# TravisWheelerLab/BATH

Measured on AMD Instinct MI355X. Metric: DP Gcells/s + residues/s through bathsearch pipeline at 1/2/4/8 MI355X, higher is better.
Workload: dtype u8/i16 integer scores (SSV: exact binary16), f32 Forward

## Files before the change

bath_amd/csrc/bath_common.hpp:

```cpp
#pragma once
#include <set>
#include <atomic>
#include <hip/hip_runtime.h>

#include <cstdint>
#include <chrono>
#include <cstdio>
#include <cstdlib>
#include <cstring>
#include <condition_variable>
#include <functional>
#include <mutex>
#include <string>
#include <thread>
#include <vector>

#include "bath_hip.h"
#include "bath_tilings.hpp"
#include "bath_slots.hpp"

namespace bath {

inline hipError_t allow_max_lds(const void *fn) {
  static std::mutex mu;
  static std::set<std::pair<int, const void *>> done;
  int dev = 0;
  (void)hipGetDevice(&dev);
  std::lock_guard<std::mutex> g(mu);
  if (done.count({dev, fn})) return hipSuccess;
  hipFuncAttributes at{};
  size_t fixed = 0;
  if (hipFuncGetAttributes(&at, fn) == hipSuccess) fixed = at.sharedSizeBytes; else (void)hipGetLastError();
  const hipError_t e = hipFuncSetAttribute(fn, hipFuncAttributeMaxDynamicSharedMemorySize, (int)(160 * 1024 - (int)std::min<size_t>(fixed, 96 * 1024)));
  if (e == hipSuccess) done.insert({dev, fn});
  return e;
}

constexpr int kKp = BATH_KP_AMINO;
constexpr int kRowReset = 29;
constexpr int kSsvRows = 30;
constexpr size_t kSsvLdsMax = 160 * 1024;
constexpr int kSsvMaxNodes = 2560;
constexpr int kStop = 27;
constexpr int kXaa = 26;
constexpr int kOrfBins = 2048;
constexpr int kOrfCursorStride = 32;
constexpr int kOrfMiscInts = (1 + kOrfCursorStride) * kOrfBins + 64;
constexpr int kFsMaxNodes = 64 * BATH_TILING_MAX(BATH_FS_COLUMNS);
constexpr int kCascadeMaxNodes = 64 * BATH_TILING_MAX(BATH_WAVE_COLUMNS);

#define BATH_HIP_TRY(ctx, call)                                                            \
  do {                                                                                     \
    hipError_t e_ = (call);                                                                \
    if (e_ != hipSuccess) {                                                                \
      (ctx)->set_error(std::string(#call) + ": " + hipGetErrorString(e_));                 \
      return BATH_EFAIL;                                                                   \
    }                                                                                      \
  } while (0)

struct DevBuf {
  void *p = nullptr;
  size_t cap = 0;
  hipError_t reserve(size_t bytes) {
    if (bytes <= cap) return hipSuccess;
    if (p) (void)hipFree(p);
    p = nullptr; cap = 0;
    size_t want = bytes + bytes / 4 + 256;
    hipError_t e = hipMalloc(&p, want);
    if (e == hipSuccess) cap = want;
    return e;
  }
  void release() { if (p) (void)hipFree(p); p = nullptr; cap = 0; }
  template <class T> T *as() const { return reinterpret_cast<T *>(p); }
};

struct HostBuf {
  void *p = nullptr;
  size_t cap = 0;
  bool coherent = false;
  hipError_t reserve(size_t bytes, bool want_coherent = false) {
    if (bytes <= cap && (coherent || !want_coherent)) return hipSuccess;
    if (p) (void)hipHostFree(p);
    p = nullptr; cap = 0;
    coherent = coherent || want_coherent;
    size_t want = bytes + bytes / 4 + 256;
    hipError_t e = hipHostMalloc(&p, want, coherent ? (hipHostMallocCoherent | hipHostMallocMapped | hipHostMallocPortable) : hipHostMallocDefault);
    if (e == hipSuccess) cap = want;
    return e;
  }
  void release() { if (p) (void)hipHostFree(p); p = nullptr; cap = 0; }
  template <class T> T *as() const { return reinterpret_cast<T *>(p); }
};

struct LanePool {
  std::mutex m;
  std::condition_variable cv_work, cv_done;
  std::vector<std::thread> th;
  std::function<void(int)> fn;
  int gen = 0, pending = 0, K = 0;
  bool stop = false;
  void loop(int id) {
    int seen = 0;
    for (;;) {
      std::function<void(int)> f;
      {
        std::unique_lock<std::mutex> l(m);
        cv_work.wait(l, [&] { return stop || (gen != seen && id < K); });
        if (stop) return;
        seen = gen; f = fn;
      }
      f(id);
      { std::lock_guard<std::mutex> l(m); if (--pending == 0) cv_done.notify_all(); }
    }
  }
  void run(int k, std::function<void(int)> f) {
    while ((int)th.size() < k) { const int id = (int)th.size(); th.emplace_back([this, id] { loop(id); }); }
    { std::lock_guard<std::mutex> l(m); fn = std::move(f); K = k; pending = k; gen++; }
    cv_work.notify_all();
    std::unique_lock<std::mutex> l(m);
    cv_done.wait(l, [&] { return pending == 0; });
  }
  ~LanePool() {
    { std::lock_guard<std::mutex> l(m); stop = true; }
    cv_work.notify_all();
    for (std::thread &t : th) t.join();
  }
};

struct StageTiming { const char *name; float ms; int64_t launches; };
struct KernelSpan { const char *name; hipEvent_t a, b; double cells, bytes; };

struct PipelineSurvivor {
  int64_t window;
  int64_t aa_off;
  int32_t strand, start;
  int32_t n;
  int32_t win_start = 0;
  int32_t fs_window = -1;
  int64_t fx_off = -1;
};

}

struct bath_hip_ctx;
namespace bath {
extern std::atomic<int> g_ctx_total, g_ctx_internal;
inline int host_contexts() { return g_ctx_total.load() - g_ctx_internal.load(); }
inline void mark_internal(bath_hip_ctx *c);
}
struct bath_hip_ctx {
  int device = 0;
  hipStream_t stream = nullptr;
  hipStream_t side_stream = nullptr;
  hipEvent_t ev_fork = nullptr, ev_join = nullptr;
  hipStream_t copy_stream = nullptr;
  hipDeviceProp_t prop{};
  int fs_strict = 1;
  int fs_odds = 0;
  int fs5_odds = 0;
  int fwd_group = 0;
  int fs_ensemble = 0;
  std::atomic<int64_t> fs_ens_bound_fallbacks{0}, fs_ens_overflow_fallbacks{0}, fs_ens_bytes_kept{0};
  int std_ensemble = 0;
  std::atomic<int64_t> std_ens_serial_fallbacks{0}, std_ens_twin_fallbacks{0}, std_ens_kernel_regions{0};
  int fs_serial = -1;
  uint64_t tabs_uid = 0;
  const void *tabs_ptr = nullptr;
  uint64_t fsw_pad_uid = 0;
  int orf_tables_id = -1;
  std::string err;
  void set_error(const std::string &m) { err = m; }
  std::vector<float> fsw_len_terms;
  bath::SlotArray<bath::Scratch, bath::DevBuf> scratch;
  bath::SlotArray<bath::Pinned, bath::HostBuf> stage;
  template <class T> int stage_upload(bath::Pinned slot, void *dst, const T *src, size_t n, hipStream_t s) {
    if (stage[slot].reserve(n * sizeof(T) + 64) != hipSuccess) { set_error("cannot allocate page-locked staging memory"); return BATH_EFAIL; }
    std::memcpy(stage[slot].p, src, n * sizeof(T));
    if (hipMemcpyAsync(dst, stage[slot].p, n * sizeof(T), hipMemcpyHostToDevice, s) != hipSuccess) { set_error("staging upload failed"); return BATH_EFAIL; }
    return BATH_OK;
  }
  bath::HostBuf results_pinned;
  bath_orf_result *d_records = nullptr;
  int64_t n_records = 0;
  std::vector<bath_orf> orfs;
  std::vector<bath_fs_window> fs_windows;
  bool keep_fwd_rows = false;
  const float *fwd_rows_kept = nullptr;
  const int64_t *fwd_rows_off = nullptr;
  bool fs_want_regions = false;
  std::vector<int64_t> fs_keep_xoff;
  std::vector<int32_t> fs_regions_all;
  std::vector<bath_fs_domain> fs_domains;
  std::string cigars;
  struct TraceRec { int64_t col_off; int32_t ncol, k1, i_first, win_start, orf_start, frameshift, d_i; };
  std::vector<TraceRec> tr_recs;
  std::vector<uint16_t> tr_codes;
  std::vector<float> tr_pp;
  void traces_clear() { tr_recs.clear(); tr_codes.clear(); tr_pp.clear(); tr_valid = false; }
  void trace_push(const uint16_t *codes, const float *pp, int ncol, int k1, int i_first, int win_start, int orf_start, int frameshift, int d_i) {
    tr_recs.push_back(TraceRec{(int64_t)tr_codes.size(), ncol, k1, i_first, win_start, orf_start, frameshift, d_i});
    tr_codes.insert(tr_codes.end(), codes, codes + ncol);
    if (pp) tr_pp.insert(tr_pp.end(), pp, pp + ncol); else tr_pp.insert(tr_pp.end(), (size_t)ncol, 0.0f);
    tr_valid = false;
  }
  bool tr_valid = false;
  std::vector<bath_domain_trace> tr_out;
  std::vector<int8_t> tr_st, tr_c;
  std::vector<int32_t> tr_k, tr_i;
  std::vector<bath::PipelineSurvivor> fs_std_orfs;
  const uint8_t *fs_std_pool = nullptr;
  std::vector<uint8_t> orf_aa;
  std::vector<bath_orf_work> orf_work;
  std::vector<bath_hmm_window> hmm_windows;
  std::vector<bath::StageTiming> timings;
  std::vector<hipEvent_t> ev_pool;
  std::vector<bath::KernelSpan> spans;
  std::vector<hipEvent_t> span_events;
  size_t span_events_used = 0;
  void spans_reset() { spans.clear(); span_events_used = 0; }
  int span_begin(const char *name, hipStream_t s, double cells, double bytes) {
    auto get = [&]() -> hipEvent_t {
      if (span_events_used == span_events.size()) { hipEvent_t e; if (hipEventCreate(&e) != hipSuccess) return nullptr; span_events.push_back(e); }
      return span_events[span_events_used++];
    };
    bath::KernelSpan k{name, get(), get(), cells, bytes};
    if (!k.a || !k.b) return -1;
    (void)hipEventRecord(k.a, s);
    spans.push_back(k);
    return (int)spans.size() - 1;
  }
  void span_end(int idx, hipStream_t s) { if (idx >= 0) (void)hipEventRecord(spans[(size_t)idx].b, s); }
  std::vector<bath_hip_ctx *> lanes;
  bath::LanePool *lane_pool = nullptr;
  hipEvent_t ev_lanes = nullptr;
  bath_hip_ctx *aux = nullptr;
  bath_hip_ctx *aux2 = nullptr;
  bath_hip_ctx *aux3 = nullptr;
  bool internal = false;
};

namespace bath {
inline void mark_internal(bath_hip_ctx *c) { if (c && !c->internal) { c->internal = true; g_ctx_internal.fetch_add(1); } }
}

struct SeqView {
  const uint8_t *data;
  const int64_t *off;
  const int32_t *len;
  int64_t n;
  const int32_t *context;
};

struct bath_hip_seqs {
  bath_hip_ctx *ctx = nullptr;
  int64_t n = 0;
  int64_t total = 0;
  int64_t total_aligned = 0;
  mutable int64_t cache_minlen = -1, cache_nres = 0, cache_max_orfs = 0;
  mutable int64_t ntiles = -1;
  mutable void *d_tile_desc = nullptr;
  mutable int32_t *d_tile_first = nullptr;
  bool is_part = false;
  int64_t first_window = 0;
  mutable std::vector<bath_hip_seqs *> parts;
  int32_t maxlen = 0;
  uint8_t *d_data = nullptr;
  int64_t *d_off = nullptr;
  int32_t *d_len = nullptr;
  int32_t *d_context = nullptr;
  uint8_t *d_packed = nullptr;
  int64_t *d_poff = nullptr;
  int64_t packed_bytes = 0;
  void *d_exc = nullptr;
  int64_t exc_cap = 0, n_exc = 0;
  hipEvent_t ev_upload = nullptr;
  bool upload_pending = false;
  std::vector<int64_t> h_off;
  std::vector<int32_t> h_len;
  std::vector<int32_t> h_context;
  SeqView view() const { return SeqView{d_data, d_off, d_len, n, d_context}; }
};

struct LenTables {
  int32_t maxL = -1;
  uint8_t *d_tjb = nullptr;
  int16_t *d_xwmove = nullptr;
  float   *d_pmove = nullptr;
  float   *d_nullsc = nullptr;
  float   *d_lt1 = nullptr;
  float   *d_lt2 = nullptr;
  float   *d_p1 = nullptr;
  std::vector<uint8_t> h_tjb;
  std::vector<int16_t> h_xwmove;
  std::vector<float> h_pmove, h_nullsc;
};

struct bath_hip_oprofile {
  bath_hip_ctx *ctx = nullptr;
  uint64_t uid = 0;
  int M = 0, max_length = 0, L0 = 0;
  float nj = 1.f;
  float evparam[BATH_NEVPARAM];
  float compo[BATH_K_AMINO];
  std::vector<uint8_t> rb;
  std::vector<int16_t> rw;
  std::vector<int16_t> tw;
  std::vector<float> rf, tf;
// ... 54 lines not shown
```

bath_amd/csrc/bath_profile.hip:

```cpp
#include <atomic>
#include <cctype>
#include <cmath>
#include <cstring>

#include "bath_common.hpp"
#include "host_model.hpp"

using namespace bath;

namespace bath {

static const double kLog2 = 0.69314718055994529;

double gumbel_surv(double x, double mu, double lambda) {
  double ey = -std::exp(-lambda * (x - mu));
  if (std::fabs(ey) < 5e-9) return -ey;
  return 1.0 - std::exp(ey);
}
double gumbel_invsurv(double p, double mu, double lambda) {
  double lp = (p < 5e-9) ? (std::pow(p, p) - 1) / p : std::log(-1. * std::log(1 - p));
  return mu - lp / lambda;
}
double exp_surv(double x, double mu, double lambda) { return (x < mu) ? 1.0 : std::exp(-lambda * (x - mu)); }

static inline uint8_t cost_u8(float scale, float sc) {
  float c = -1.0f * roundf(scale * sc);
  return (c > 255.) ? 255 : (uint8_t)(int)c;
}
static inline uint8_t cost_u8_biased(float scale, uint8_t bias, float sc) {
  float c = -1.0f * roundf(scale * sc);
  return (c > 255 - bias) ? 255 : (uint8_t)((int)c + bias);
}
static inline int16_t score_i16(float scale, float sc) {
  float v = roundf(scale * sc);
  if (v >= 32767.0) return 32767;
  if (v <= -32768.0) return -32768;
  return (int16_t)v;
}

void bias_filter_eo(const float *compo, float eo[kKp][2]) {
  for (int x = 0; x < 20; x++) { eo[x][0] = kAminoBg[x] / kAminoBg[x]; eo[x][1] = compo[x] / kAminoBg[x]; }
  for (int x : {20, 27, 28}) eo[x][0] = eo[x][1] = 1.0f;
  for (int x = 21; x <= 26; x++)
    for (int s = 0; s < 2; s++) {
      float num = 0.f, den = 0.f;
      for (int y = 0; y < 20; y++)
        if (amino_degen_has(x, y)) { num += (s == 0 ? kAminoBg[y] : compo[y]); den += kAminoBg[y]; }
      eo[x][s] = den > 0.f ? num / den : 0.f;
    }
}

template <class T>
static hipError_t upload(T **dst, const T *src, size_t n, hipStream_t st) {
  hipError_t e = hipMalloc((void **)dst, n * sizeof(T) + 64);
  if (e != hipSuccess) return e;
  return hipMemcpyAsync(*dst, src, n * sizeof(T), hipMemcpyHostToDevice, st);
}

int build_len_tables(const bath_hip_oprofile *om, int maxL) {
  std::lock_guard<std::mutex> lock(om->grow_mu);
  LenTables &lt = om->lt;
  if (maxL <= lt.maxL) return BATH_OK;
  bath_hip_ctx *ctx = om->ctx;
  int n = std::max(maxL, 4096) + 1;
  for (void *p : {(void *)lt.d_tjb, (void *)lt.d_xwmove, (void *)lt.d_pmove, (void *)lt.d_nullsc, (void *)lt.d_lt1, (void *)lt.d_lt2, (void *)lt.d_p1})
    if (p) om->retired.push_back(p);
  lt.d_tjb = nullptr; lt.d_xwmove = nullptr; lt.d_pmove = nullptr; lt.d_nullsc = nullptr; lt.d_lt1 = nullptr; lt.d_lt2 = nullptr; lt.d_p1 = nullptr;
  lt.h_tjb.resize(n); lt.h_xwmove.resize(n); lt.h_pmove.resize(n); lt.h_nullsc.resize(n);
  std::vector<float> lt1(n), lt2(n), p1v(n);
  for (int L = 0; L < n; L++) {
    lt.h_tjb[L] = cost_u8(om->scale_b, logf(3.0f / (float)(L + 3)));
    float pmove = (2.0f + om->nj) / ((float)L + 2.0f + om->nj);
    lt.h_pmove[L] = pmove;
    lt.h_xwmove[L] = score_i16(om->scale_w, logf(pmove));
    float p1 = (float)L / (float)(L + 1);
    p1v[L] = p1;
    lt.h_nullsc[L] = (float)((float)L * std::log((double)p1) + std::log(1. - p1));
    lt1[L] = (float)L * logf(p1);
    lt2[L] = logf((float)(1. - p1));
  }
  BATH_HIP_TRY(ctx, upload(&lt.d_tjb, lt.h_tjb.data(), n, ctx->stream));
  BATH_HIP_TRY(ctx, upload(&lt.d_xwmove, lt.h_xwmove.data(), n, ctx->stream));
  BATH_HIP_TRY(ctx, upload(&lt.d_pmove, lt.h_pmove.data(), n, ctx->stream));
  BATH_HIP_TRY(ctx, upload(&lt.d_nullsc, lt.h_nullsc.data(), n, ctx->stream));
  BATH_HIP_TRY(ctx, upload(&lt.d_lt1, lt1.data(), n, ctx->stream));
  BATH_HIP_TRY(ctx, upload(&lt.d_lt2, lt2.data(), n, ctx->stream));
  BATH_HIP_TRY(ctx, upload(&lt.d_p1, p1v.data(), n, ctx->stream));
  BATH_HIP_TRY(ctx, hipStreamSynchronize(ctx->stream));
  lt.maxL = n - 1;
  return BATH_OK;
}

}

int bath_hip_oprofile::ensure_len_tables(int maxL) const { return bath::build_len_tables(this, maxL); }


namespace bath { std::atomic<int> g_ctx_total{0}, g_ctx_internal{0}; }

extern "C" int bath_hip_init(int device, bath_hip_ctx **out) {
  *out = nullptr;
  int ndev = 0;
  if (hipGetDeviceCount(&ndev) != hipSuccess || ndev <= 0) return BATH_ENODEVICE;
  if (device < 0 || device >= ndev) return BATH_EINVAL;
  bath_hip_ctx *ctx = new bath_hip_ctx();
  ctx->device = device;
  if (const char *e = std::getenv("BATH_HIP_SYNC")) {
    static const bool once = [&] {
      (void)hipSetDevice(device);
      const unsigned fl = (e[0] == 'b') ? hipDeviceScheduleBlockingSync : (e[0] == 'y') ? hipDeviceScheduleYield : hipDeviceScheduleSpin;
      if (hipSetDeviceFlags(fl) != hipSuccess) (void)hipGetLastError();
      return true;
    }();
    (void)once;
  }
  if (hipSetDevice(device) != hipSuccess || hipGetDeviceProperties(&ctx->prop, device) != hipSuccess ||
      hipStreamCreateWithFlags(&ctx->stream, hipStreamNonBlocking) != hipSuccess) {
    delete ctx;
    return BATH_ENODEVICE;
  }
  bath::g_ctx_total.fetch_add(1);
  *out = ctx;
  return BATH_OK;
}

extern "C" void bath_hip_finalize(bath_hip_ctx *ctx) {
  if (!ctx) return;
  bath::g_ctx_total.fetch_sub(1);
  if (ctx->internal) bath::g_ctx_internal.fetch_sub(1);
  (void)hipSetDevice(ctx->device);
  (void)hipStreamSynchronize(ctx->stream);
  delete ctx->lane_pool; ctx->lane_pool = nullptr;
  for (bath_hip_ctx *lane : ctx->lanes) bath_hip_finalize(lane);
  ctx->lanes.clear();
  if (ctx->ev_lanes) (void)hipEventDestroy(ctx->ev_lanes);
  if (ctx->aux) { bath_hip_finalize(ctx->aux); ctx->aux = nullptr; }
  if (ctx->aux2) { bath_hip_finalize(ctx->aux2); ctx->aux2 = nullptr; }
  if (ctx->aux3) { bath_hip_finalize(ctx->aux3); ctx->aux3 = nullptr; }
  for (auto &b : ctx->scratch) b.release();
  for (auto &b : ctx->stage) b.release();
  ctx->results_pinned.release();
  for (auto e : ctx->ev_pool) (void)hipEventDestroy(e);
  for (auto e : ctx->span_events) (void)hipEventDestroy(e);
  if (ctx->ev_fork) (void)hipEventDestroy(ctx->ev_fork);
  if (ctx->ev_join) (void)hipEventDestroy(ctx->ev_join);
  if (ctx->copy_stream) (void)hipStreamDestroy(ctx->copy_stream);
  if (ctx->side_stream) (void)hipStreamDestroy(ctx->side_stream);
  (void)hipStreamDestroy(ctx->stream);
  delete ctx;
}

extern "C" int bath_hip_trim(bath_hip_ctx *ctx) {
  if (!ctx) return BATH_EINVAL;
  BATH_HIP_TRY(ctx, hipSetDevice(ctx->device));
  BATH_HIP_TRY(ctx, hipStreamSynchronize(ctx->stream));
  delete ctx->lane_pool; ctx->lane_pool = nullptr;
  for (bath_hip_ctx *lane : ctx->lanes) bath_hip_finalize(lane);
  ctx->lanes.clear();
  if (ctx->aux) { bath_hip_finalize(ctx->aux); ctx->aux = nullptr; }
  if (ctx->aux2) { bath_hip_finalize(ctx->aux2); ctx->aux2 = nullptr; }
  if (ctx->aux3) { bath_hip_finalize(ctx->aux3); ctx->aux3 = nullptr; }
  if (ctx->copy_stream) { (void)hipStreamSynchronize(ctx->copy_stream); (void)hipStreamDestroy(ctx->copy_stream); ctx->copy_stream = nullptr; }
  if (ctx->side_stream) {
    (void)hipStreamSynchronize(ctx->side_stream); (void)hipStreamDestroy(ctx->side_stream); ctx->side_stream = nullptr;
    if (ctx->ev_fork) { (void)hipEventDestroy(ctx->ev_fork); ctx->ev_fork = nullptr; }
    if (ctx->ev_join) { (void)hipEventDestroy(ctx->ev_join); ctx->ev_join = nullptr; }
  }
  ctx->fs_std_orfs.clear(); ctx->fs_std_pool = nullptr; ctx->fs_keep_xoff.clear(); ctx->fs_regions_all.clear();
  ctx->d_records = nullptr; ctx->n_records = 0;
  return BATH_OK;
}

extern "C" const char *bath_hip_last_error(const bath_hip_ctx *ctx) { return ctx ? ctx->err.c_str() : "no context"; }

extern "C" int bath_hip_synchronize(bath_hip_ctx *ctx) {
  BATH_HIP_TRY(ctx, hipSetDevice(ctx->device));
  BATH_HIP_TRY(ctx, hipStreamSynchronize(ctx->stream));
  return BATH_OK;
}

extern "C" void *bath_hip_stream(bath_hip_ctx *ctx) { return (void *)ctx->stream; }
extern "C" int bath_hip_kernel_times(bath_hip_ctx *ctx, int max, bath_kernel_time *out) {
  if (!ctx || !out) return 0;
  int n = 0;
  for (const bath_hip_ctx *c : {(const bath_hip_ctx *)ctx, (const bath_hip_ctx *)ctx->aux, (const bath_hip_ctx *)ctx->aux2, (const bath_hip_ctx *)ctx->aux3}) {
    if (!c) continue;
    for (const bath::KernelSpan &k : c->spans) {
      float ms = 0.f;
      if (hipEventSynchronize(k.b) != hipSuccess || hipEventElapsedTime(&ms, k.a, k.b) != hipSuccess) continue;
      int i = 0;
      while (i < n && out[i].name != k.name) i++;
      if (i == n) { if (n == max) continue; out[n++] = bath_kernel_time{k.name, 0.f, 0, 0.0, 0.0}; }
      out[i].ms += ms; out[i].launches++; out[i].cells += k.cells; out[i].bytes += k.bytes;
    }
  }
  return n;
}
extern "C" int bath_hip_set_fs_serial(bath_hip_ctx *ctx, int on) {
  if (!ctx) return BATH_EINVAL;
  ctx->fs_serial = on < 0 ? -1 : (on ? 1 : 0);
  return BATH_OK;
}

extern "C" int bath_hip_set_fs_strict(bath_hip_ctx *ctx, int on) {
  if (!ctx) return BATH_EINVAL;
  ctx->fs_strict = on ? 1 : 0;
  if (!on && ctx->aux3) { bath_hip_finalize(ctx->aux3); ctx->aux3 = nullptr; }
  for (bath_hip_ctx *l : ctx->lanes) l->fs_strict = ctx->fs_strict;
  return BATH_OK;
}

extern "C" int bath_hip_set_fwd_group(bath_hip_ctx *ctx, int mode) {
  if (!ctx) return BATH_EINVAL;
  if (mode < 0 || mode > 2) { ctx->set_error("bath_hip_set_fwd_group: mode must be 0, 1 or 2"); return BATH_EINVAL; }
  ctx->fwd_group = mode;
  for (bath_hip_ctx *l : ctx->lanes) l->fwd_group = mode;
  return BATH_OK;
}

extern "C" int bath_hip_set_fs_odds(bath_hip_ctx *ctx, int on) {
  if (!ctx) return BATH_EINVAL;
  ctx->fs_odds = on ? 1 : 0;
  for (bath_hip_ctx *l : ctx->lanes) l->fs_odds = ctx->fs_odds;
  return BATH_OK;
}

extern "C" int bath_hip_set_fs5_odds(bath_hip_ctx *ctx, int on) {
  if (!ctx) return BATH_EINVAL;
  ctx->fs5_odds = on ? 1 : 0;
  for (bath_hip_ctx *l : ctx->lanes) l->fs5_odds = ctx->fs5_odds;
  return BATH_OK;
}

extern "C" int bath_hip_set_fs_ensemble(bath_hip_ctx *ctx, int mode) {
  if (!ctx) return BATH_EINVAL;
  if (mode != BATH_ENSEMBLE_SERIAL && mode != BATH_ENSEMBLE_STREAMS_HOST && mode != BATH_ENSEMBLE_STREAMS_DEVICE) { ctx->set_error("bath_hip_set_fs_ensemble: unknown mode " + std::to_string(mode)); return BATH_EINVAL; }
  ctx->fs_ensemble = mode;
  for (bath_hip_ctx *l : ctx->lanes) l->fs_ensemble = mode;
  return BATH_OK;
}

extern "C" int bath_hip_set_std_ensemble(bath_hip_ctx *ctx, int mode) {
  if (!ctx) return BATH_EINVAL;
  if (mode != BATH_ENSEMBLE_SERIAL && mode != BATH_ENSEMBLE_STREAMS_HOST && mode != BATH_ENSEMBLE_STREAMS_DEVICE) { ctx->set_error("bath_hip_set_std_ensemble: unknown mode " + std::to_string(mode)); return BATH_EINVAL; }
  ctx->std_ensemble = mode;
  for (bath_hip_ctx *l : ctx->lanes) l->std_ensemble = mode;
  if (ctx->aux) ctx->aux->std_ensemble = mode;
  return BATH_OK;
}

extern "C" int bath_hip_std_ensemble_counters(bath_hip_ctx *ctx, int64_t *serial_fallbacks, int64_t *twin_fallbacks, int64_t *kernel_regions) {
  if (!ctx) return BATH_EINVAL;
  int64_t s = 0, t = 0, k = 0;
  for (const bath_hip_ctx *c : {(const bath_hip_ctx *)ctx, (const bath_hip_ctx *)ctx->aux}) {
    if (!c) continue;
    s += c->std_ens_serial_fallbacks.load(); t += c->std_ens_twin_fallbacks.load(); k += c->std_ens_kernel_regions.load();
  }
  if (serial_fallbacks) *serial_fallbacks = s;
  if (twin_fallbacks) *twin_fallbacks = t;
  if (kernel_regions) *kernel_regions = k;
  return BATH_OK;
}

extern "C" int bath_hip_fs_ensemble_counters(bath_hip_ctx *ctx, int64_t *bound_fallbacks, int64_t *overflow_fallbacks, int64_t *matrix_bytes_kept) {
  if (!ctx) return BATH_EINVAL;
  int64_t b = 0, o = 0, k = 0;
  for (const bath_hip_ctx *c : {(const bath_hip_ctx *)ctx, (const bath_hip_ctx *)ctx->aux2}) {
    if (!c) continue;
    b += c->fs_ens_bound_fallbacks.load(); o += c->fs_ens_overflow_fallbacks.load(); k += c->fs_ens_bytes_kept.load();
  }
  if (bound_fallbacks) *bound_fallbacks = b;
  if (overflow_fallbacks) *overflow_fallbacks = o;
  if (matrix_bytes_kept) *matrix_bytes_kept = k;
  return BATH_OK;
}

extern "C" int bath_selftest_compute_units(const bath_hip_ctx *ctx) { return ctx ? ctx->prop.multiProcessorCount : 0; }


extern "C" void bath_hip_oprofile_destroy(bath_hip_oprofile *om) {
  if (!om) return;
  for (void *p : {(void *)om->d_emit, (void *)om->d_ssv, (void *)om->d_msv, (void *)om->d_rb, (void *)om->d_rw, (void *)om->d_tw, (void *)om->d_rf, (void *)om->d_tf,
                  (void *)om->d_bias_eo, (void *)om->d_compo_terms, (void *)om->d_vit_rw, (void *)om->d_vit_tw2, (void *)om->d_vit_rank, (void *)om->lt.d_tjb, (void *)om->lt.d_xwmove, (void *)om->lt.d_pmove,
                  (void *)om->lt.d_nullsc, (void *)om->lt.d_lt1, (void *)om->lt.d_lt2, (void *)om->lt.d_p1, (void *)om->d_cons, (void *)om->d_msc, (void *)om->d_tsc, (void *)om->d_rfb, (void *)om->d_tfb})
    if (p) (void)hipFree(p);
  for (void *p : om->retired) (void)hipFree(p);
  delete om;
}

extern "C" int bath_hip_oprofile_set_consensus(bath_hip_oprofile *om, const char *consensus) {
  if (!om || !consensus) return BATH_EINVAL;
  bath_hip_ctx *ctx = om->ctx;
  static const char syms[] = "ACDEFGHIKLMNPQRSTVWY-BJZOUX*~";
  om->consensus.assign((size_t)om->M + 2, ' ');
  om->cons_digital.assign((size_t)om->M + 1, 255);
  for (int k = 1; k <= om->M && consensus[k]; k++) {
    om->consensus[(size_t)k] = consensus[k];
    const char *q = std::strchr(syms, std::toupper((unsigned char)consensus[k]));
    if (q) om->cons_digital[(size_t)k] = (uint8_t)(q - syms);
  }
  if (!om->d_cons) BATH_HIP_TRY(ctx, hipMalloc(&om->d_cons, (size_t)om->M + 1));
  BATH_HIP_TRY(ctx, hipMemcpy(om->d_cons, om->cons_digital.data(), (size_t)om->M + 1, hipMemcpyHostToDevice));
  return BATH_OK;
}

extern "C" int bath_hip_oprofile_M(const bath_hip_oprofile *om) { return om->M; }

extern "C" int bath_hip_oprofile_convert(bath_hip_ctx *ctx, const bath_profile *gm, bath_hip_oprofile **ret) {
  *ret = nullptr;
  const int M = gm->M;
  if (M < 1) { ctx->set_error("profile has no nodes"); return BATH_EINVAL; }
  BATH_HIP_TRY(ctx, hipSetDevice(ctx->device));
  const size_t W = (size_t)M + 1;
  auto msc = [&](int k, int x) { return gm->rsc[(size_t)x * W * 2 + 2 * k]; };
  auto tsc = [&](int k, int s) { return gm->tsc[(size_t)k * 8 + s]; };
  enum { MM, IM, DM, BM, MD, DD, MI, II };

  bath_hip_oprofile *om = new bath_hip_oprofile();
  { static std::atomic<uint64_t> next_uid{1}; om->uid = next_uid.fetch_add(1); }
// ... 381 lines not shown
```

bath_amd/csrc/bath_viterbi.hip:

```cpp
#include <algorithm>
#include <cstdlib>
#include <functional>

#include "bath_common.hpp"
#include "bath_kernels.hpp"
#include "bath_launch.hpp"

using namespace bath;

namespace bath {

__device__ __forceinline__ s16x2 pk_adds(s16x2 a, s16x2 b) { return __builtin_elementwise_add_sat(a, b); }
__device__ __forceinline__ s16x2 pk_max(s16x2 a, s16x2 b) { return __builtin_elementwise_max(a, b); }
__device__ __forceinline__ s16x2 as_s2(unsigned v) { return __builtin_bit_cast(s16x2, v); }
__device__ __forceinline__ unsigned as_u(s16x2 v) { return __builtin_bit_cast(unsigned, v); }

struct VitLaneTables {
  const int16_t *rw;
  int rw_pitch_bytes;
  const uint32_t *tw2;
  const int16_t *rank;
};

struct VitLaneConsts {
  int M, base_w, xwE_loop, xwE_move, Q8;
  float scale_w;
  double invP_vit, invP_msv;
  float scale_b;
  int base_b, tec_b, bias_b;
};

typedef uint32_t u32x16 __attribute__((ext_vector_type(16)));

template <int NR>
__global__ __launch_bounds__(256, 1) void vit_lane_kernel(SeqView sq, VitLaneTables tb, const uint32_t *__restrict__ tw2g, VitLaneConsts c, const int16_t *__restrict__ xwmove_tab,
                                                          const uint8_t *__restrict__ tjb_tab, const int32_t *__restrict__ todo, int64_t ntodo,
                                                          const int *__restrict__ ntodo_dev, const int *__restrict__ skip_dev, float *__restrict__ sc, int32_t *__restrict__ status,
                                                          const float *__restrict__ filtersc, const uint8_t *__restrict__ ssv_scores,
                                                          WindowRec *__restrict__ wins, int *__restrict__ win_count, int win_cap, int32_t *__restrict__ kminmax) {
  extern __shared__ __attribute__((aligned(16))) char lds[];
  char *s_rw = lds;
  int16_t *s_rank = reinterpret_cast<int16_t *>(lds + 30 * tb.rw_pitch_bytes);
  {
    const uint32_t *src = reinterpret_cast<const uint32_t *>(tb.rw);
    uint32_t *dst = reinterpret_cast<uint32_t *>(s_rw);
    for (int i = threadIdx.x; i < 30 * tb.rw_pitch_bytes / 4; i += blockDim.x) dst[i] = src[i];
    for (int i = threadIdx.x; i < 2 * NR; i += blockDim.x) s_rank[i] = tb.rank[i];
  }
  __syncthreads();
  if (ntodo_dev) ntodo = *ntodo_dev;
  const int64_t t = (int64_t)blockIdx.x * blockDim.x + threadIdx.x + (skip_dev ? *skip_dev : 0);
  if (t - (threadIdx.x & 63) >= ntodo) return;
  const bool live = t < ntodo;
  const int64_t sid = live ? (todo ? (int64_t)todo[t] : t) : (todo ? (int64_t)todo[0] : 0);
  const int L = live ? sq.len[sid] : 0;
  const uint8_t *s = sq.data + sq.off[sid];
  const int Lw = wave_max_i32(L);
  const bool do_win = (wins != nullptr);
  const int M = c.M;

  const int xw_move = xwmove_tab[L];
  int sc_thresh = 0, sc_ext_thresh = 0, skip_until = 0, kmin = 1 << 30, kmax = 0;
  if (do_win && live) {
    const double fsc = (double)filtersc[sid];
    sc_thresh = (int)(int16_t)(int)ceil(((fsc + 0.69314718055994529 * c.invP_vit + 3.0) * (double)c.scale_w) -
                                        (double)(float)c.xwE_move - (double)(float)xw_move + (double)(float)c.base_w);
    sc_ext_thresh = (int)ceil(((fsc + 0.69314718055994529 * c.invP_msv + 3.0) * (double)c.scale_b) + c.base_b + c.tec_b + (int)tjb_tab[L]);
  }
  const s16x2 NEG = {-32768, -32768};
  s16x2 Mr[NR], Ir[NR], Dr[NR];
#pragma unroll
  for (int r = 0; r < NR; r++) Mr[r] = Ir[r] = Dr[r] = NEG;
  int xN = c.base_w;
  int xB = (int16_t)(xN + xw_move);
  int xJ = -32768, xC = -32768;
  bool overflow = false;
  short ePrev = -32768;

  uint32_t wnext = (0 < L) ? *reinterpret_cast<const uint32_t *>(s) : 0x1d1d1d1du;
  for (int i0 = 0; i0 < Lw; i0 += 4) {
    const uint32_t w = wnext;
    wnext = (i0 + 4 < L) ? *reinterpret_cast<const uint32_t *>(s + i0 + 4) : 0x1d1d1d1du;
#pragma unroll 1
    for (int j = 0; j < 4; j++) {
      const int i = i0 + j + 1;
      const bool on = (i <= L) && !overflow;
      int x = (w >> (8 * j)) & 0xff;
      x = (i <= L) ? min(x, kKp - 1) : 29;
      const char *rowbase = s_rw + x * tb.rw_pitch_bytes;
      const s16x2 xBv = {(short)xB, (short)xB};
      s16x2 xEv = NEG;
      unsigned pM = (as_u(Mr[NR - 1]) << 16) | 0x8000u, pI = (as_u(Ir[NR - 1]) << 16) | 0x8000u, pD = (as_u(Dr[NR - 1]) << 16) | 0x8000u;
      s16x2 dpk = NEG;
      s16x2 cpk = {(short)-32768, ePrev};
      int twz = 0;
      asm volatile("" : "+s"(twz));
      const uint32_t *tw = tw2g + twz;
      u32x16 t_c, t_n;
      int4 e_c = *reinterpret_cast<const int4 *>(rowbase), e_n = e_c;
      asm volatile("s_load_dwordx16 %0, %1, 0x0" : "=s"(t_c) : "s"(tw));
#pragma unroll
      for (int r = 0; r < NR; r += 2) {
        asm volatile("s_waitcnt lgkmcnt(0)" ::: "memory");
        __builtin_amdgcn_sched_barrier(0);
        if ((r & 3) == 0 && r + 4 < NR) e_n = *reinterpret_cast<const int4 *>(rowbase + 4 * (r + 4));
        if (r + 2 < NR) asm volatile("s_load_dwordx16 %0, %1, %2" : "=s"(t_n) : "s"(tw), "i"((r + 2) * 32));
        __builtin_amdgcn_sched_barrier(0);
        const unsigned em[2] = {(r & 3) ? (unsigned)e_c.z : (unsigned)e_c.x, (r & 3) ? (unsigned)e_c.w : (unsigned)e_c.y};
#pragma unroll
        for (int q = 0; q < 2; q++) {
          const int rr = r + q;
          const unsigned tMM = t_c[8 * q + 0], tIM = t_c[8 * q + 1], tDM = t_c[8 * q + 2], tBM = t_c[8 * q + 3];
          const unsigned tMD = t_c[8 * q + 4], tDD = t_c[8 * q + 5], tMI = t_c[8 * q + 6], tII = t_c[8 * q + 7];
          const unsigned oM = as_u(Mr[rr]), oI = as_u(Ir[rr]);
          const unsigned oD = as_u(pk_max(Dr[rr], cpk));
          cpk = pk_adds(cpk, as_s2(tDD));
          const s16x2 ms = as_s2(pM), is = as_s2(pI), ds = as_s2(pD);
          s16x2 sv = pk_adds(xBv, as_s2(tBM));
          sv = pk_max(sv, pk_adds(ms, as_s2(tMM)));
          sv = pk_max(sv, pk_adds(is, as_s2(tIM)));
          sv = pk_max(sv, pk_adds(ds, as_s2(tDM)));
          sv = pk_adds(sv, as_s2(em[q]));
          Ir[rr] = pk_max(pk_adds(as_s2(oM), as_s2(tMI)), pk_adds(as_s2(oI), as_s2(tII)));
          const s16x2 dcv = pk_adds(sv, as_s2(tMD));
          xEv = pk_max(xEv, sv);
          Mr[rr] = sv;
          Dr[rr] = dpk;
          dpk = pk_max(dcv, pk_adds(dpk, as_s2(tDD)));
          pM = oM; pI = oI; pD = oD;
        }
        if (r + 2 < NR) t_c = t_n;
        if ((r & 3) == 2 && r + 2 < NR) e_c = e_n;
        asm volatile("" : "+v"(Mr[r]), "+v"(Mr[r + 1]), "+v"(Ir[r]), "+v"(Ir[r + 1]), "+v"(Dr[r]), "+v"(Dr[r + 1]), "+v"(dpk), "+v"(cpk), "+v"(xEv));
        __builtin_amdgcn_sched_barrier(0);
      }
      ePrev = dpk.x;
      if (on) {
        const int xE = max((int)xEv.x, (int)xEv.y);
        if (xE >= 32767) overflow = true;
        else {
          xN = (int16_t)(xN + 0);
          xC = (int16_t)max(xC + 0, xE + c.xwE_move);
          xJ = (int16_t)max(xJ + 0, xE + c.xwE_loop);
          xB = (int16_t)max(xJ + xw_move, xN + xw_move);
          if (do_win && i > skip_until && xE >= sc_thresh) {
            int rank = 32767;
#pragma unroll
            for (int r = 0; r < NR; r++) {
              if ((int)Mr[r].x == xE) rank = min(rank, (int)s_rank[2 * r]);
              if ((int)Mr[r].y == xE) rank = min(rank, (int)s_rank[2 * r + 1]);
            }
            const int k_start = (rank / 8) + c.Q8 * (rank % 8) + 1;
            int max_k_end = k_start, max_i_end = i, sc_ext = sc_ext_thresh, max_sc_ext = sc_ext, since = 0;
            int kk = k_start + 1, nn = i + 1;
            while (kk <= M && nn <= L) {
              sc_ext += c.bias_b - (int)ssv_scores[(size_t)kk * kKp + min((int)s[nn - 1], kKp - 1)];
              if (sc_ext >= max_sc_ext) { max_sc_ext = sc_ext; max_k_end = kk; max_i_end = nn; since = 0; }
              else if (++since == 5) break;
              kk++; nn++;
            }
            const int slot = atomicAdd(win_count, 1);
            if (slot < win_cap) wins[slot] = WindowRec{(int32_t)sid, i, max_k_end, max_k_end - k_start + 1, 0.0f};
            kmax = max(kmax, max_k_end);
            kmin = min(kmin, k_start);
            skip_until = max_i_end;
          }
        }
      }
    }
  }
  if (live) {
    if (overflow) { sc[sid] = INFINITY; status[sid] = BATH_ERANGE; }
    else if (xC > -32768) {
      float r = (float)xC + (float)xw_move - (float)c.base_w;
      r /= c.scale_w;
      r = (float)((double)r - 3.0);
      sc[sid] = r; status[sid] = BATH_OK;
    } else { sc[sid] = -INFINITY; status[sid] = BATH_OK; }
    if (do_win && kminmax) { kminmax[2 * sid] = kmin; kminmax[2 * sid + 1] = kmax; }
  }
}

constexpr int kLenBins = 2048;
constexpr int kVitLongTarget = 128;
__device__ __forceinline__ void len_block_range(int n, int &lo, int &hi) {
  const int per = (n + (int)gridDim.x - 1) / (int)gridDim.x;
  lo = min(n, (int)blockIdx.x * per); hi = min(n, lo + per);
}
__global__ __launch_bounds__(256) void len_hist_kernel(const int32_t *__restrict__ todo, const int *__restrict__ ntodo_dev, const int32_t *__restrict__ len,
                                                       int *__restrict__ hist) {
  __shared__ int s_cnt[kLenBins];
  for (int i = threadIdx.x; i < kLenBins; i += blockDim.x) s_cnt[i] = 0;
  __syncthreads();
  int lo, hi;
  len_block_range(*ntodo_dev, lo, hi);
  for (int j = lo + threadIdx.x; j < hi; j += blockDim.x) atomicAdd(&s_cnt[min(len[todo[j]], kLenBins - 1)], 1);
  __syncthreads();
  for (int i = threadIdx.x; i < kLenBins; i += blockDim.x) if (s_cnt[i]) atomicAdd(&hist[i], s_cnt[i]);
}
__global__ __launch_bounds__(256) void len_scan_kernel(int *__restrict__ hist ) {
  constexpr int kPer = kLenBins / 256;
  __shared__ int s_wsum[4];
  const int tid = threadIdx.x, lane = tid & 63, wv = tid >> 6;
  int c[kPer], sum = 0;
#pragma unroll
  for (int k = 0; k < kPer; k++) { c[k] = hist[kLenBins - 1 - (kPer * tid + k)]; sum += c[k]; }
  int x = sum;
#pragma unroll
  for (int d = 1; d < 64; d <<= 1) { const int y = __shfl_up(x, d, 64); if (lane >= d) x += y; }
  if (lane == 63) s_wsum[wv] = x;
  __syncthreads();
  int run = x - sum;
#pragma unroll
  for (int u = 0; u < 4; u++) run += u < wv ? s_wsum[u] : 0;
#pragma unroll
  for (int k = 0; k < kPer; k++) { hist[kLenBins - 1 - (kPer * tid + k)] = run; run += c[k]; }
}
__global__ __launch_bounds__(256) void len_scatter_kernel(const int32_t *__restrict__ todo, const int *__restrict__ ntodo_dev, const int32_t *__restrict__ len,
                                                          int *__restrict__ cursor, int32_t *__restrict__ sorted) {
  __shared__ int s_cnt[kLenBins];
  for (int i = threadIdx.x; i < kLenBins; i += blockDim.x) s_cnt[i] = 0;
  __syncthreads();
  int lo, hi;
  len_block_range(*ntodo_dev, lo, hi);
  for (int j = lo + threadIdx.x; j < hi; j += blockDim.x) atomicAdd(&s_cnt[min(len[todo[j]], kLenBins - 1)], 1);
  __syncthreads();
  for (int i = threadIdx.x; i < kLenBins; i += blockDim.x) { const int c = s_cnt[i]; if (c) s_cnt[i] = atomicAdd(&cursor[i], c); }
  __syncthreads();
  for (int j = lo + threadIdx.x; j < hi; j += blockDim.x) {
    const int cnd = todo[j];
    sorted[atomicAdd(&s_cnt[min(len[cnd], kLenBins - 1)], 1)] = cnd;
  }
}

int vit_lane_supported(const bath_hip_oprofile *om) { return om->vit_NR > 0; }

const int *len_sort_count_longer(const int *d_bins, int T) { return d_bins + std::min(T + 1, kLenBins - 1); }

int launch_len_sort(bath_hip_ctx *ctx, const int32_t *d_todo, const int *d_ntodo, const int32_t *d_len, int *d_bins, int32_t *d_sorted) {
  BATH_HIP_TRY(ctx, hipMemsetAsync(d_bins, 0, kLenBins * sizeof(int), ctx->stream));
  hipLaunchKernelGGL(len_hist_kernel, dim3(256), dim3(256), 0, ctx->stream, d_todo, d_ntodo, d_len, d_bins);
  hipLaunchKernelGGL(len_scan_kernel, dim3(1), dim3(256), 0, ctx->stream, d_bins);
  hipLaunchKernelGGL(len_scatter_kernel, dim3(256), dim3(256), 0, ctx->stream, d_todo, d_ntodo, d_len, d_bins, d_sorted);
  BATH_HIP_TRY(ctx, hipGetLastError());
  return BATH_OK;
}

extern "C" int bath_selftest_len_sort(bath_hip_ctx *ctx, int n, const int32_t *lens, int T, int32_t *sorted, int32_t *n_longer) {
  if (!ctx || n < 0 || (n > 0 && (!lens || !sorted)) || !n_longer) return BATH_EINVAL;
  BATH_HIP_TRY(ctx, hipSetDevice(ctx->device));
  const size_t m = (size_t)std::max(n, 1);
  int32_t *d = nullptr;
  BATH_HIP_TRY(ctx, hipMalloc((void **)&d, (3 * m + kLenBins + 1) * sizeof(int32_t)));
  int32_t *d_len = d, *d_todo = d + m, *d_sorted = d + 2 * m, *d_bins = d + 3 * m, *d_n = d_bins + kLenBins;
  std::vector<int32_t> todo(m);
  for (size_t i = 0; i < m; i++) todo[i] = (int32_t)i;
  hipError_t e = hipSuccess;
  if (n > 0) e = hipMemcpy(d_len, lens, (size_t)n * sizeof(int32_t), hipMemcpyHostToDevice);
  if (e == hipSuccess) e = hipMemcpy(d_todo, todo.data(), m * sizeof(int32_t), hipMemcpyHostToDevice);
  if (e == hipSuccess) e = hipMemcpy(d_n, &n, sizeof(int32_t), hipMemcpyHostToDevice);
  int st = e == hipSuccess ? launch_len_sort(ctx, d_todo, d_n, d_len, d_bins, d_sorted) : BATH_EFAIL;
  if (st == BATH_OK) e = hipStreamSynchronize(ctx->stream);
  if (st == BATH_OK && e == hipSuccess && n > 0) e = hipMemcpy(sorted, d_sorted, (size_t)n * sizeof(int32_t), hipMemcpyDeviceToHost);
  if (st == BATH_OK && e == hipSuccess) e = hipMemcpy(n_longer, len_sort_count_longer(d_bins, T), sizeof(int32_t), hipMemcpyDeviceToHost);
  (void)hipFree(d);
  if (st == BATH_OK && e != hipSuccess) { ctx->set_error(std::string("bath_selftest_len_sort: ") + hipGetErrorString(e)); st = BATH_EFAIL; }
  return st;
}

int launch_vit_lane(bath_hip_ctx *ctx, const bath_hip_oprofile *om, SeqView v, const int32_t *d_todo, int64_t ntodo, const int *ntodo_dev,
                    float *d_sc, int32_t *d_status, const VitWindowArgs *wa, const int *skip_dev) {
  if (ntodo == 0) return BATH_OK;
  VitLaneTables tb{om->d_vit_rw, om->vit_rw_pitch, om->d_vit_tw2, om->d_vit_rank};
  VitLaneConsts c{};
  c.M = om->M; c.base_w = om->base_w; c.xwE_loop = om->xw_E[0]; c.xwE_move = om->xw_E[1]; c.Q8 = std::max(2, ((om->M - 1) / 8) + 1);
  c.scale_w = om->scale_w; c.scale_b = om->scale_b; c.base_b = om->base_b; c.tec_b = om->tec_b; c.bias_b = om->bias_b;
  const float *fsc = nullptr; const uint8_t *ssv = nullptr; WindowRec *wins = nullptr; int *wc = nullptr; int cap = 0; int32_t *kmm = nullptr;
  if (wa) { c.invP_vit = wa->invP_vit; c.invP_msv = wa->invP_msv; fsc = wa->d_filtersc; ssv = wa->d_ssv_scores; wins = (WindowRec *)wa->d_wins; wc = wa->d_win_count; cap = wa->win_cap; kmm = wa->d_kminmax; }
  const int NRv = om->vit_NR;
  const size_t shmem = (size_t)30 * om->vit_rw_pitch + (size_t)2 * NRv * 2 + 16;
  const int blocks = (int)((ntodo + 255) / 256);
  bool launched = false;
#define BATH_VITL_CASE(N, ...)                                                                                                         \
  if (!launched && NRv == N) {                                                                                                         \
    hipLaunchKernelGGL(vit_lane_kernel<N>, dim3(blocks), dim3(256), shmem, ctx->stream, v, tb, tb.tw2, c, om->lt.d_xwmove, om->lt.d_tjb, d_todo, ntodo, \
                       ntodo_dev, skip_dev, d_sc, d_status, fsc, ssv, wins, wc, cap, kmm);                                                       \
    launched = true;                                                                                                                   \
  }
  BATH_VIT_LANE_NR(BATH_VITL_CASE)
#undef BATH_VITL_CASE
  if (!launched) { ctx->set_error("lane-per-target Viterbi kernel: unsupported model length"); return BATH_EINVAL; }
  BATH_HIP_TRY(ctx, hipGetLastError());
  return BATH_OK;
}

int64_t lane_min_nt() {
  static const int64_t v = [] { const char *e = std::getenv("BATH_HIP_LANE_MIN_NT"); return e ? std::atoll(e) : (int64_t)150'000'000; }();
  return v;
}

const char *vit_lane_kernel_name(const bath_hip_oprofile *om) {
#define BATH_VITL_NAME(N, ...) if (om->vit_NR == N) return "vit_lane_kernel<" #N ">";
  BATH_VIT_LANE_NR(BATH_VITL_NAME)
#undef BATH_VITL_NAME
  return "vit_lane_kernel<?>";
}

int launch_vit_sorted(bath_hip_ctx *ctx, const bath_hip_oprofile *om, SeqView v, const int32_t *d_todo, int64_t cap, const int *d_ntodo, const int32_t *d_len,
                      int *d_bins, int32_t *d_sorted, float *d_sc, int32_t *d_status, const VitWindowArgs *wa, const std::function<int(hipStream_t)> &beside) {
  int st;
  if ((st = launch_len_sort(ctx, d_todo, d_ntodo, d_len, d_bins, d_sorted)) != BATH_OK) return st;
  if (!ctx->side_stream) {
    BATH_HIP_TRY(ctx, hipStreamCreateWithFlags(&ctx->side_stream, hipStreamNonBlocking));
    BATH_HIP_TRY(ctx, hipEventCreateWithFlags(&ctx->ev_fork, hipEventDisableTiming));
    BATH_HIP_TRY(ctx, hipEventCreateWithFlags(&ctx->ev_join, hipEventDisableTiming));
  }
  const int *d_nlong = len_sort_count_longer(d_bins, kVitLongTarget);
  BATH_HIP_TRY(ctx, hipEventRecord(ctx->ev_fork, ctx->stream));
  BATH_HIP_TRY(ctx, hipStreamWaitEvent(ctx->side_stream, ctx->ev_fork, 0));
  {
    hipStream_t main_stream = ctx->stream;
    ctx->stream = ctx->side_stream;
    st = launch_vit_wave(ctx, om, v, d_sorted, cap, d_sc, d_status, wa, d_nlong);
    ctx->stream = main_stream;
    if (st != BATH_OK) return st;
    if (beside && (st = beside(ctx->side_stream)) != BATH_OK) return st;
  }
  BATH_HIP_TRY(ctx, hipEventRecord(ctx->ev_join, ctx->side_stream));
  if ((st = launch_vit_lane(ctx, om, v, d_sorted, cap, d_ntodo, d_sc, d_status, wa, d_nlong)) != BATH_OK) return st;
  BATH_HIP_TRY(ctx, hipStreamWaitEvent(ctx->stream, ctx->ev_join, 0));
  return BATH_OK;
}

}
```

Baseline: 217.6 billion.

## Drop per-row D registers in Viterbi lane kernel and run beside-work on own stream

The lane Viterbi kernel no longer keeps a D-state register array per row. The previous row's D values are carried in a rolling qd chain, and only the last row's D is kept across iterations. This cuts VGPR pressure, so kernels with NR<=80 now request two waves per EU through launch_bounds. Separately, the 'beside' callback now runs on a new second side stream instead of being serialised after the wave kernel. That lets it overlap with both the wave and lane kernels, at the cost of another stream and event to manage.

```diff
diff --git a/bath_amd/csrc/bath_common.hpp b/bath_amd/csrc/bath_common.hpp
--- a/bath_amd/csrc/bath_common.hpp
+++ b/bath_amd/csrc/bath_common.hpp
@@ -153,6 +153,8 @@
   hipStream_t stream = nullptr;
   hipStream_t side_stream = nullptr;
   hipEvent_t ev_fork = nullptr, ev_join = nullptr;
+  hipStream_t side_stream2 = nullptr;
+  hipEvent_t ev_join2 = nullptr;
   hipStream_t copy_stream = nullptr;
   hipDeviceProp_t prop{};
   int fs_strict = 1;
diff --git a/bath_amd/csrc/bath_profile.hip b/bath_amd/csrc/bath_profile.hip
--- a/bath_amd/csrc/bath_profile.hip
+++ b/bath_amd/csrc/bath_profile.hip
@@ -144,8 +144,10 @@
   for (auto e : ctx->span_events) (void)hipEventDestroy(e);
   if (ctx->ev_fork) (void)hipEventDestroy(ctx->ev_fork);
   if (ctx->ev_join) (void)hipEventDestroy(ctx->ev_join);
+  if (ctx->ev_join2) (void)hipEventDestroy(ctx->ev_join2);
   if (ctx->copy_stream) (void)hipStreamDestroy(ctx->copy_stream);
   if (ctx->side_stream) (void)hipStreamDestroy(ctx->side_stream);
+  if (ctx->side_stream2) (void)hipStreamDestroy(ctx->side_stream2);
   (void)hipStreamDestroy(ctx->stream);
   delete ctx;
 }
@@ -165,6 +167,10 @@
     (void)hipStreamSynchronize(ctx->side_stream); (void)hipStreamDestroy(ctx->side_stream); ctx->side_stream = nullptr;
     if (ctx->ev_fork) { (void)hipEventDestroy(ctx->ev_fork); ctx->ev_fork = nullptr; }
     if (ctx->ev_join) { (void)hipEventDestroy(ctx->ev_join); ctx->ev_join = nullptr; }
+  }
+  if (ctx->side_stream2) {
+    (void)hipStreamSynchronize(ctx->side_stream2); (void)hipStreamDestroy(ctx->side_stream2); ctx->side_stream2 = nullptr;
+    if (ctx->ev_join2) { (void)hipEventDestroy(ctx->ev_join2); ctx->ev_join2 = nullptr; }
   }
   ctx->fs_std_orfs.clear(); ctx->fs_std_pool = nullptr; ctx->fs_keep_xoff.clear(); ctx->fs_regions_all.clear();
   ctx->d_records = nullptr; ctx->n_records = 0;
diff --git a/bath_amd/csrc/bath_viterbi.hip b/bath_amd/csrc/bath_viterbi.hip
--- a/bath_amd/csrc/bath_viterbi.hip
+++ b/bath_amd/csrc/bath_viterbi.hip
@@ -32,8 +32,10 @@
 
 typedef uint32_t u32x16 __attribute__((ext_vector_type(16)));
 
+constexpr int kVitLaneTwoWavesNR = 80;
+
 template <int NR>
-__global__ __launch_bounds__(256, 1) void vit_lane_kernel(SeqView sq, VitLaneTables tb, const uint32_t *__restrict__ tw2g, VitLaneConsts c, const int16_t *__restrict__ xwmove_tab,
+__global__ __launch_bounds__(256, NR <= kVitLaneTwoWavesNR ? 2 : 1) void vit_lane_kernel(SeqView sq, VitLaneTables tb, const uint32_t *__restrict__ tw2g, VitLaneConsts c, const int16_t *__restrict__ xwmove_tab,
                                                           const uint8_t *__restrict__ tjb_tab, const int32_t *__restrict__ todo, int64_t ntodo,
                                                           const int *__restrict__ ntodo_dev, const int *__restrict__ skip_dev, float *__restrict__ sc, int32_t *__restrict__ status,
                                                           const float *__restrict__ filtersc, const uint8_t *__restrict__ ssv_scores,
@@ -68,14 +70,14 @@
     sc_ext_thresh = (int)ceil(((fsc + 0.69314718055994529 * c.invP_msv + 3.0) * (double)c.scale_b) + c.base_b + c.tec_b + (int)tjb_tab[L]);
   }
   const s16x2 NEG = {-32768, -32768};
-  s16x2 Mr[NR], Ir[NR], Dr[NR];
-#pragma unroll
-  for (int r = 0; r < NR; r++) Mr[r] = Ir[r] = Dr[r] = NEG;
+  s16x2 Mr[NR], Ir[NR];
+#pragma unroll
+  for (int r = 0; r < NR; r++) Mr[r] = Ir[r] = NEG;
   int xN = c.base_w;
   int xB = (int16_t)(xN + xw_move);
   int xJ = -32768, xC = -32768;
   bool overflow = false;
-  short ePrev = -32768;
+  short ePrev = -32768, dNPrev = -32768;
 
   uint32_t wnext = (0 < L) ? *reinterpret_cast<const uint32_t *>(s) : 0x1d1d1d1du;
   for (int i0 = 0; i0 < Lw; i0 += 4) {
@@ -90,9 +92,11 @@
       const char *rowbase = s_rw + x * tb.rw_pitch_bytes;
       const s16x2 xBv = {(short)xB, (short)xB};
       s16x2 xEv = NEG;
-      unsigned pM = (as_u(Mr[NR - 1]) << 16) | 0x8000u, pI = (as_u(Ir[NR - 1]) << 16) | 0x8000u, pD = (as_u(Dr[NR - 1]) << 16) | 0x8000u;
+      unsigned pM = (as_u(Mr[NR - 1]) << 16) | 0x8000u, pI = (as_u(Ir[NR - 1]) << 16) | 0x8000u;
+      unsigned pD = ((unsigned)(unsigned short)dNPrev << 16) | 0x8000u;
       s16x2 dpk = NEG;
-      s16x2 cpk = {(short)-32768, ePrev};
+      s16x2 qd = {(short)-32768, ePrev};
+      short dNcur = -32768;
       int twz = 0;
       asm volatile("" : "+s"(twz));
       const uint32_t *tw = tw2g + twz;
@@ -113,8 +117,8 @@
           const unsigned tMM = t_c[8 * q + 0], tIM = t_c[8 * q + 1], tDM = t_c[8 * q + 2], tBM = t_c[8 * q + 3];
           const unsigned tMD = t_c[8 * q + 4], tDD = t_c[8 * q + 5], tMI = t_c[8 * q + 6], tII = t_c[8 * q + 7];
           const unsigned oM = as_u(Mr[rr]), oI = as_u(Ir[rr]);
-          const unsigned oD = as_u(pk_max(Dr[rr], cpk));
-          cpk = pk_adds(cpk, as_s2(tDD));
+          const unsigned oD = as_u(qd);
+          qd = pk_max(pk_adds(as_s2(oM), as_s2(tMD)), pk_adds(qd, as_s2(tDD)));
           const s16x2 ms = as_s2(pM), is = as_s2(pI), ds = as_s2(pD);
           s16x2 sv = pk_adds(xBv, as_s2(tBM));
           sv = pk_max(sv, pk_adds(ms, as_s2(tMM)));
@@ -125,16 +129,16 @@
           const s16x2 dcv = pk_adds(sv, as_s2(tMD));
           xEv = pk_max(xEv, sv);
           Mr[rr] = sv;
-          Dr[rr] = dpk;
+          if (rr == NR - 1) dNcur = dpk.x;
           dpk = pk_max(dcv, pk_adds(dpk, as_s2(tDD)));
           pM = oM; pI = oI; pD = oD;
         }
         if (r + 2 < NR) t_c = t_n;
         if ((r & 3) == 2 && r + 2 < NR) e_c = e_n;
-        asm volatile("" : "+v"(Mr[r]), "+v"(Mr[r + 1]), "+v"(Ir[r]), "+v"(Ir[r + 1]), "+v"(Dr[r]), "+v"(Dr[r + 1]), "+v"(dpk), "+v"(cpk), "+v"(xEv));
+        asm volatile("" : "+v"(Mr[r]), "+v"(Mr[r + 1]), "+v"(Ir[r]), "+v"(Ir[r + 1]), "+v"(dpk), "+v"(qd), "+v"(xEv));
         __builtin_amdgcn_sched_barrier(0);
       }
-      ePrev = dpk.x;
+      ePrev = dpk.x; dNPrev = dNcur;
       if (on) {
         const int xE = max((int)xEv.x, (int)xEv.y);
         if (xE >= 32767) overflow = true;
@@ -315,6 +319,11 @@
     BATH_HIP_TRY(ctx, hipEventCreateWithFlags(&ctx->ev_fork, hipEventDisableTiming));
     BATH_HIP_TRY(ctx, hipEventCreateWithFlags(&ctx->ev_join, hipEventDisableTiming));
   }
+  const bool abreast = beside && !ctx->internal;
+  if (abreast && !ctx->side_stream2) {
+    BATH_HIP_TRY(ctx, hipStreamCreateWithFlags(&ctx->side_stream2, hipStreamNonBlocking));
+    BATH_HIP_TRY(ctx, hipEventCreateWithFlags(&ctx->ev_join2, hipEventDisableTiming));
+  }
   const int *d_nlong = len_sort_count_longer(d_bins, kVitLongTarget);
   BATH_HIP_TRY(ctx, hipEventRecord(ctx->ev_fork, ctx->stream));
   BATH_HIP_TRY(ctx, hipStreamWaitEvent(ctx->side_stream, ctx->ev_fork, 0));
@@ -324,11 +333,17 @@
     st = launch_vit_wave(ctx, om, v, d_sorted, cap, d_sc, d_status, wa, d_nlong);
     ctx->stream = main_stream;
     if (st != BATH_OK) return st;
-    if (beside && (st = beside(ctx->side_stream)) != BATH_OK) return st;
+    if (beside && !abreast && (st = beside(ctx->side_stream)) != BATH_OK) return st;
   }
   BATH_HIP_TRY(ctx, hipEventRecord(ctx->ev_join, ctx->side_stream));
+  if (abreast) {
+    BATH_HIP_TRY(ctx, hipStreamWaitEvent(ctx->side_stream2, ctx->ev_fork, 0));
+    if ((st = beside(ctx->side_stream2)) != BATH_OK) return st;
+    BATH_HIP_TRY(ctx, hipEventRecord(ctx->ev_join2, ctx->side_stream2));
+  }
   if ((st = launch_vit_lane(ctx, om, v, d_sorted, cap, d_ntodo, d_sc, d_status, wa, d_nlong)) != BATH_OK) return st;
   BATH_HIP_TRY(ctx, hipStreamWaitEvent(ctx->stream, ctx->ev_join, 0));
+  if (abreast) BATH_HIP_TRY(ctx, hipStreamWaitEvent(ctx->stream, ctx->ev_join2, 0));
   return BATH_OK;
 }
 
```

After: 218.9 billion (median of 2 runs). About the same (+0.6%).

## Convert lane Viterbi kernel to a persistent grid-stride loop over targets

Applied to the files above, without the earlier changes.

Caps the Viterbi lane kernel grid at a few blocks per compute unit and has each block loop over target chunks with a grid stride. The LDS table copy then happens once per block instead of once per 256 targets, and blocks past the device-side work count exit before loading tables. It also pins the window-threshold constants into scalar registers with an empty asm barrier and switches indices to 32-bit. The trade-off is less tail balancing when target lengths vary, since each block now processes a fixed strided set of chunks.

```diff
diff --git a/bath_amd/csrc/bath_viterbi.hip b/bath_amd/csrc/bath_viterbi.hip
--- a/bath_amd/csrc/bath_viterbi.hip
+++ b/bath_amd/csrc/bath_viterbi.hip
@@ -38,6 +38,9 @@
                                                           const int *__restrict__ ntodo_dev, const int *__restrict__ skip_dev, float *__restrict__ sc, int32_t *__restrict__ status,
                                                           const float *__restrict__ filtersc, const uint8_t *__restrict__ ssv_scores,
                                                           WindowRec *__restrict__ wins, int *__restrict__ win_count, int win_cap, int32_t *__restrict__ kminmax) {
+  const uint32_t n = (uint32_t)(ntodo_dev ? max(0, min(*ntodo_dev, (int)ntodo)) : (int)ntodo);
+  const uint32_t skip = skip_dev ? (uint32_t)*skip_dev : 0u;
+  if (blockIdx.x * 256u + skip >= n) return;
   extern __shared__ __attribute__((aligned(16))) char lds[];
   char *s_rw = lds;
   int16_t *s_rank = reinterpret_cast<int16_t *>(lds + 30 * tb.rw_pitch_bytes);
@@ -48,11 +51,12 @@
     for (int i = threadIdx.x; i < 2 * NR; i += blockDim.x) s_rank[i] = tb.rank[i];
   }
   __syncthreads();
-  if (ntodo_dev) ntodo = *ntodo_dev;
-  const int64_t t = (int64_t)blockIdx.x * blockDim.x + threadIdx.x + (skip_dev ? *skip_dev : 0);
-  if (t - (threadIdx.x & 63) >= ntodo) return;
-  const bool live = t < ntodo;
-  const int64_t sid = live ? (todo ? (int64_t)todo[t] : t) : (todo ? (int64_t)todo[0] : 0);
+  const uint32_t stride = __builtin_amdgcn_readfirstlane(gridDim.x * 256u), wave0 = __builtin_amdgcn_readfirstlane(threadIdx.x & ~63u);
+  for (uint32_t first = blockIdx.x * 256u + skip; first < n; first += stride) {
+  if (first + wave0 >= n) break;
+  const uint32_t t = first + threadIdx.x;
+  const bool live = t < n;
+  const int64_t sid = live ? (todo ? (int64_t)todo[t] : (int64_t)t) : (todo ? (int64_t)todo[0] : 0);
   const int L = live ? sq.len[sid] : 0;
   const uint8_t *s = sq.data + sq.off[sid];
   const int Lw = wave_max_i32(L);
@@ -62,10 +66,14 @@
   const int xw_move = xwmove_tab[L];
   int sc_thresh = 0, sc_ext_thresh = 0, skip_until = 0, kmin = 1 << 30, kmax = 0;
   if (do_win && live) {
+    double invP_vit = c.invP_vit, invP_msv = c.invP_msv;
+    float scale_w = c.scale_w, scale_b = c.scale_b;
+    int xwE_move = c.xwE_move, base_w = c.base_w, base_b = c.base_b, tec_b = c.tec_b;
+    asm volatile("" : "+s"(invP_vit), "+s"(invP_msv), "+s"(scale_w), "+s"(scale_b), "+s"(xwE_move), "+s"(base_w), "+s"(base_b), "+s"(tec_b));
     const double fsc = (double)filtersc[sid];
-    sc_thresh = (int)(int16_t)(int)ceil(((fsc + 0.69314718055994529 * c.invP_vit + 3.0) * (double)c.scale_w) -
-                                        (double)(float)c.xwE_move - (double)(float)xw_move + (double)(float)c.base_w);
-    sc_ext_thresh = (int)ceil(((fsc + 0.69314718055994529 * c.invP_msv + 3.0) * (double)c.scale_b) + c.base_b + c.tec_b + (int)tjb_tab[L]);
+    sc_thresh = (int)(int16_t)(int)ceil(((fsc + 0.69314718055994529 * invP_vit + 3.0) * (double)scale_w) -
+                                        (double)(float)xwE_move - (double)(float)xw_move + (double)(float)base_w);
+    sc_ext_thresh = (int)ceil(((fsc + 0.69314718055994529 * invP_msv + 3.0) * (double)scale_b) + base_b + tec_b + (int)tjb_tab[L]);
   }
   const s16x2 NEG = {-32768, -32768};
   s16x2 Mr[NR], Ir[NR], Dr[NR];
@@ -179,6 +187,7 @@
     } else { sc[sid] = -INFINITY; status[sid] = BATH_OK; }
     if (do_win && kminmax) { kminmax[2 * sid] = kmin; kminmax[2 * sid + 1] = kmax; }
   }
+  }
 }
 
 constexpr int kLenBins = 2048;
@@ -268,9 +277,18 @@
   return st;
 }
 
+constexpr int kVitGridRounds = 4;
+static int vit_lane_grid(const bath_hip_ctx *ctx, int64_t ntodo) {
+  const char *e = std::getenv("BATH_HIP_TEST_VIT_GRID");
+  const int forced = e ? std::atoi(e) : 0;
+  const int64_t bound = forced > 0 ? forced : (int64_t)std::max(1, ctx->prop.multiProcessorCount) * kVitGridRounds;
+  return (int)std::min<int64_t>((ntodo + 255) / 256, bound);
+}
+
 int launch_vit_lane(bath_hip_ctx *ctx, const bath_hip_oprofile *om, SeqView v, const int32_t *d_todo, int64_t ntodo, const int *ntodo_dev,
                     float *d_sc, int32_t *d_status, const VitWindowArgs *wa, const int *skip_dev) {
   if (ntodo == 0) return BATH_OK;
+  if (ntodo < 0 || ntodo > (int64_t)INT32_MAX) { ctx->set_error("lane-per-target Viterbi kernel: the work list's indices are 32-bit"); return BATH_EINVAL; }
   VitLaneTables tb{om->d_vit_rw, om->vit_rw_pitch, om->d_vit_tw2, om->d_vit_rank};
   VitLaneConsts c{};
   c.M = om->M; c.base_w = om->base_w; c.xwE_loop = om->xw_E[0]; c.xwE_move = om->xw_E[1]; c.Q8 = std::max(2, ((om->M - 1) / 8) + 1);
@@ -279,7 +297,7 @@
   if (wa) { c.invP_vit = wa->invP_vit; c.invP_msv = wa->invP_msv; fsc = wa->d_filtersc; ssv = wa->d_ssv_scores; wins = (WindowRec *)wa->d_wins; wc = wa->d_win_count; cap = wa->win_cap; kmm = wa->d_kminmax; }
   const int NRv = om->vit_NR;
   const size_t shmem = (size_t)30 * om->vit_rw_pitch + (size_t)2 * NRv * 2 + 16;
-  const int blocks = (int)((ntodo + 255) / 256);
+  const int blocks = vit_lane_grid(ctx, ntodo);
   bool launched = false;
 #define BATH_VITL_CASE(N, ...)                                                                                                         \
   if (!launched && NRv == N) {                                                                                                         \
```

Result: slower. 215.2 billion before, 212.7 billion after (-1.2%).
